# LANL-Bioinformatics/KWAGE

Hardware: AMD Instinct MI355X
Metric: G k-mer·sample bit-tests/sec (+ achieved HBM GB/s of the gather kernel in `roofline`) (higher is better)
Workload: dtype u32

## Files before the change

kwage_amd/csrc/engine.hip:

```cpp
#include <hip/hip_runtime.h>
#include <hip/hip_ext.h>

#include <algorithm>
#include <chrono>
#include <cmath>
#include <cstdio>
#include <cctype>
#include <cstring>
#include <new>
#include <string>
#include <thread>
#include <vector>

#include <unistd.h>

#include "host.hpp"
#include "engine_state.hpp"
#include "kernels.hpp"

using namespace kwage;


struct TuningName { const char *name; int64_t Tuning::*field; };
static const TuningName TUNING_NAMES[] = {
// ... 78 lines not shown
	chunk_q.reserve(n);
	chunk_t0.reserve(n);
	for(uint32_t i = 0; i < n; ++i){
		const uint64_t npos = L->h_pos_off[i + 1] - L->h_pos_off[i];
		const bool is_long = npos && (1ull << host_table_log2(npos)) > KM_LDS_SLOTS;
		if(!is_long || npos <= KM_CHUNK){ chunk_q.push_back(i); chunk_t0.push_back(0); continue; }
		L->multi_chunk = true;
		for(uint64_t t0 = 0; t0 < npos; t0 += KM_CHUNK){ chunk_q.push_back(i); chunk_t0.push_back(t0); }
	}
	if(chunk_q.size() > 0x7FFFFFFFull){ return fail(KWAGE_ERR_ARG, "batch too large for one k-mer launch"); }
	L->n_chunks = chunk_q.size();
	L->pool = &b->ctx->batch_pool;
	HIP_TRY(L->pool->take(std::max<size_t>(chunk_q.size(), 1)*sizeof(uint32_t), (void**)&L->d_chunk_q, &L->cap_chunk_q));
	HIP_TRY(L->pool->take(std::max<size_t>(chunk_q.size(), 1)*sizeof(uint64_t), (void**)&L->d_chunk_t0, &L->cap_chunk_t0));
	HIP_TRY(L->pool->take(((size_t)n + 1)*sizeof(uint64_t), (void**)&L->d_pos_off, &L->cap_pos_off));
	HIP_TRY(L->pool->take(std::max<size_t>(n, 1)*sizeof(uint64_t), (void**)&L->d_tab_off, &L->cap_tab_off));
	hipStream_t us = b->ctx->upload_stream;
	if(L->n_chunks){
		HIP_TRY(hipMemcpyAsync(L->d_chunk_q, chunk_q.data(), chunk_q.size()*sizeof(uint32_t), hipMemcpyHostToDevice, us));
		HIP_TRY(hipMemcpyAsync(L->d_chunk_t0, chunk_t0.data(), chunk_t0.size()*sizeof(uint64_t), hipMemcpyHostToDevice, us));
	}
	HIP_TRY(hipMemcpyAsync(L->d_pos_off, L->h_pos_off.data(), ((size_t)n + 1)*sizeof(uint64_t), hipMemcpyHostToDevice, us));
	if(n){ HIP_TRY(hipMemcpyAsync(L->d_tab_off, tab_off.data(), (size_t)n*sizeof(uint64_t), hipMemcpyHostToDevice, us)); }
	HIP_TRY(hipStreamSynchronize(us));
	L->total_pos = L->h_pos_off[n];
	L->max_pos = maxp;
	L->table_slots = slots;
	*out = L.get();
	b->layouts.push_back(std::move(L));
	return KWAGE_OK;
}

int launch_kmer_stage(Slot *sl, const kwage_params &p, kwage_batch *b, const KmerLayout *L, float threshold,
                      uint32_t *d_rows, uint64_t *d_kmers)
{
	int rc = layout_result(sl, b->n, 0, false);
	if(rc){ return rc; }
	if(L->table_slots){
		if((rc = sl->tables.reserve(L->table_slots*sizeof(uint64_t)))){ return rc; }
		HIP_TRY(hipMemsetAsync(sl->tables.p, 0xFF, L->table_slots*sizeof(uint64_t), sl->stream));
	}
	HIP_TRY(hipMemsetAsync(sl->d_counters, 0, 4*sizeof(uint64_t), sl->stream));
	if(b->n == 0){ return KWAGE_OK; }

	KmerArgs a;
	a.seqs = b->d_seqs;
	a.seq_off = b->d_seq_off;
	a.pos_off = L->d_pos_off;
	a.tab_off = L->d_tab_off;
	a.g_tables = (unsigned long long*)sl->tables.p;
	a.k = p.kmer_len;
	a.num_hash = p.num_hash;
	a.row_mask = (p.log_2_filter_len >= 32) ? 0xFFFFFFFFu : ((1u << p.log_2_filter_len) - 1u);
	a.threshold = threshold;
	a.complete_match = (threshold == 1.0f) ? 1 : 0;
	a.rows = d_rows;
	a.kmers_out = d_kmers;
	a.nkmer = sl->d_nkmer;
	a.qthr = sl->d_qthr;
	a.total_kmers = nullptr;
	a.shared_lg = 0;
	a.bloom_bits = nullptr;
	a.chunk_q = L->d_chunk_q;
	a.chunk_t0 = L->d_chunk_t0;
	if(L->multi_chunk){
		HIP_TRY(hipMemsetAsync(sl->d_nkmer, 0, (size_t)b->n*sizeof(uint32_t), sl->stream));
	}
	uint32_t slots = 64;
	while(slots < KM_LDS_SLOTS && slots < 2*L->max_pos){ slots *= 2; }
	a.lds_slots = slots;
	const uint32_t threads = (L->max_pos <= 192) ? 64 : (L->max_pos <= 768) ? 128 : KM_THREADS;
	hipLaunchKernelGGL(kmer_kernel, dim3((uint32_t)L->n_chunks), dim3(threads), (size_t)slots*sizeof(uint64_t), sl->stream, a);
	HIP_TRY(hipGetLastError());
	if(L->multi_chunk){
		hipLaunchKernelGGL(kmer_finish_kernel, dim3((b->n + 255)/256), dim3(256), 0, sl->stream, a, b->n);
		HIP_TRY(hipGetLastError());
	}
	return KWAGE_OK;
}

struct StageEvents { hipEvent_t start = nullptr, stop = nullptr; };

#define KW_GATHER_LAUNCH(ge, first, last, kernel, grid, block, lds, stream, ...) \
	hipExtLaunchKernelGGL(kernel, grid, block, (uint32_t)(lds), stream, (first) ? (ge).start : nullptr, (last) ? (ge).stop : nullptr, 0u, __VA_ARGS__)

static const uint32_t WALK_MIN_ROWS_PER_WAVE = 64;
static const uint32_t WALK_WAVES_PER_CU = 8;

uint32_t search_blocks(const SearchArgs &a)
{
	const uint64_t tiles = (uint64_t)a.n_queries*a.segs*a.chunks;
	return (uint32_t)((tiles + 3)/4);
}

struct WalkShape { uint32_t wgs, wg_waves; size_t lds; };
static const size_t WALK_PAD_LDS = 100*1024;

WalkShape walk_shape(const Tuning &tn, uint64_t want_waves, uint64_t ncu)
{
	WalkShape w;
	const bool pinned = tn.walk_one_wg_per_cu && want_waves == ncu*WALK_WG_WAVES;
	w.wg_waves = pinned ? (uint32_t)WALK_WG_WAVES : 4u;
	w.wgs = (uint32_t)((want_waves + w.wg_waves - 1)/w.wg_waves);
	w.lds = pinned ? WALK_PAD_LDS : 0;
	return w;
}
// ... 184 lines not shown
	ra.seg_rows = (uint32_t)std::max<uint64_t>(ra.seg_rows, (max_rows + 65535)/65536);
	ra.min_rows = (uint32_t)std::max<int64_t>(tn.refine_min_rows, 1);
	ra.max_groups = (uint32_t)std::min<int64_t>(std::max<int64_t>(tn.refine_max_groups, 0), 16);
	uint64_t items = std::min<uint64_t>(std::max<uint64_t>(8ull*a.n_queries, 1u << 16), 1u << 20);
	items = std::max<uint64_t>(std::min<uint64_t>(items, (256ull << 20)/item_bytes), 1024);
	uint64_t units = std::min<uint64_t>(std::max<uint64_t>(32*total_rows/ra.seg_rows, 1u << 18), 1u << 25);
	if(unit_bytes){ units = std::max<uint64_t>(std::min<uint64_t>(units, (512ull << 20)/unit_bytes), 4096); }
	if(tn.refine_list_cap > 0){ items = units = (uint64_t)std::min<int64_t>(tn.refine_list_cap, 1 << 20); }
	uint64_t clusters = items;
	if(exact_units){ clusters = exact_clusters; items = exact_items; units = exact_units; }
	if(exact_units && tn.refine_list_cap > 0){ clusters = items = units = (uint64_t)std::min<int64_t>(tn.refine_list_cap, 1 << 20); }
	const uint64_t tiles_per_wave = (tiles + screen_waves - 1)/std::max<uint64_t>(screen_waves, 1);
	auto list = [&](uint64_t cap, uint64_t stat_max, uint64_t chunk_max) {
		RefineList ls;
		ls.cap = (uint32_t)cap;
		ls.stat = (tn.refine_static && !exact_units) ? (uint32_t)std::min<uint64_t>(stat_max, cap/2/std::max<uint64_t>(screen_waves, 1)) : 0u;
		ls.base = (uint32_t)(ls.stat*screen_waves);
		ls.chunk = exact_units ? 1u : (uint32_t)std::max<uint64_t>(1, std::min<uint64_t>(chunk_max, tiles_per_wave/4));
		return ls;
	};
	ra.lc = list(clusters, 32, 32);
	ra.li = list(items, 64, 64);
	ra.lu = list(units, 256, 256);
	if((rc = sl->ref_counters.reserve(8*sizeof(uint32_t)))){ return rc; }
	if((rc = sl->ref_clusters.reserve(clusters*sizeof(RefineCluster)))){ return rc; }
	if((rc = sl->ref_masks.reserve(items*item_bytes))){ return rc; }
	if((rc = sl->ref_units.reserve(units*sizeof(RefineUnit)))){ return rc; }
	if(unit_bytes && (rc = sl->ref_slab.reserve(units*unit_bytes))){ return rc; }
	ra.counters = (uint32_t*)sl->ref_counters.p;
	ra.clusters = (RefineCluster*)sl->ref_clusters.p;
	ra.masks = (uint32_t*)sl->ref_masks.p;
	ra.units = (RefineUnit*)sl->ref_units.p;
	ra.slab = (uint32_t*)sl->ref_slab.p;
	HIP_TRY(hipMemsetAsync(ra.counters, 0, 8*sizeof(uint32_t), gs));
	sl->ref_base[0] = ra.lc.base; sl->ref_base[1] = ra.li.base; sl->ref_base[2] = ra.lu.base;
	sl->ref_cap[0] = ra.lc.cap; sl->ref_cap[1] = ra.li.cap; sl->ref_cap[2] = ra.lu.cap;
	ra.queue_batch = (uint32_t)std::max<uint64_t>(1, std::min<uint64_t>(16, tiles/(8*std::max<uint64_t>(screen_waves, 1))));
	ra.check_every = (tn.count_screen_check == 16 || tn.count_screen_check == 32 || tn.count_screen_check == 64) ? (uint32_t)tn.count_screen_check : 8u;
	out->refine_wgs = (uint32_t)(ncu*8);
	out->emit_wgs = (uint32_t)(ncu*4);
	return KWAGE_OK;
}

uint32_t count_screen_blocks_per_cu(uint32_t planes, uint32_t nh)
{
	static int cache[3][5] = {};
	const int pi = (planes <= 7) ? 0 : (planes <= 10) ? 1 : 2, ni = (int)std::min(std::max(nh, 1u), 5u) - 1;
	if(cache[pi][ni] == 0){
		int nb = 0;
		hipError_t e = hipErrorUnknown;
#define KWAGE_OCC_NH(P, N) case N: e = hipOccupancyMaxActiveBlocksPerMultiprocessor(&nb, count_screen_kernel<P, N>, SEARCH_THREADS, 0); break;
#define KWAGE_OCC_P(I, P) case I: switch(ni + 1){ KWAGE_OCC_NH(P, 1) KWAGE_OCC_NH(P, 2) KWAGE_OCC_NH(P, 3) KWAGE_OCC_NH(P, 4) default: KWAGE_OCC_NH(P, 5) } break;
		switch(pi){ KWAGE_OCC_P(0, 7) KWAGE_OCC_P(1, 10) default: KWAGE_OCC_P(2, 14) }
#undef KWAGE_OCC_P
#undef KWAGE_OCC_NH
		if(e != hipSuccess || nb <= 0){ (void)hipGetLastError(); nb = 2; }
		cache[pi][ni] = nb;
	}
	return (uint32_t)cache[pi][ni];
}

int launch_search_stage(Slot *sl, kwage_group *g, kwage_batch *b, const KmerLayout *L, float threshold, uint32_t flags,
                        kwage_hit *d_hits, uint64_t cap, unsigned long long *hit_count, hipStream_t gs, const StageEvents &ge)
{
	const Tuning &tn = g->ctx->tune;
	const uint64_t ncu = (uint64_t)std::max(g->ctx->ncu, 1);
	SearchArgs a;
// ... 329 lines not shown
				case 20: rc = launch_count_combine<20>(a, seg_planes, gs, ge); break;
				default: rc = launch_count_combine<32>(a, seg_planes, gs, ge); break;
			}
			if(rc){ return rc; }
		}
	}
	HIP_TRY(hipGetLastError());
	return KWAGE_OK;
}

static const uint64_t SPEC_HITS = 8192;
static const uint64_t SORT_SCRATCH_KEEP = 1ull << 30;

struct SearchOutcome {
	uint64_t staged_hits = 0;
	uint64_t n_hits = 0;
	uint64_t total_kmers = 0;
	float kmer_ms = 0, search_ms = 0;
	uint32_t launches = 0;
	char kernel_name[64] = "";
};

int enqueue_search_and_copy(Slot *sl)
{
	int rc;
	kwage_group *g = sl->g;
	kwage_batch *b = sl->b;
	const bool timing = (sl->flags & KWAGE_SEARCH_TIMING) != 0;
	const bool own = (sl->ext_hits == nullptr && sl->ext_cap == 0);
	const uint64_t cap = own ? sl->hit_cap : sl->ext_cap;
	kwage_hit *d_hits = own ? sl->d_hits : sl->ext_hits;
	if(b->n && g->num_columns){
		hipStream_t gs = g->ctx->gather_stream;
		if(sl->n_runs){ HIP_TRY(hipMemsetAsync(sl->runs.p, 0, sl->n_runs*sizeof(unsigned long long), sl->stream)); }
		HIP_TRY(hipEventRecord(sl->kmer_done, sl->stream));
		HIP_TRY(hipStreamWaitEvent(gs, sl->kmer_done, 0));
		if(sl->append && sl->append_reset){ HIP_TRY(hipMemsetAsync(sl->ext_count, 0, sizeof(uint64_t), gs)); }
		const bool ride = g->ctx->tune.ext_launch_events != 0;
		StageEvents ge;
		if(ride){ ge.start = timing ? sl->ev[2] : nullptr; ge.stop = sl->gather_done; }
		else if(timing){ HIP_TRY(hipEventRecord(sl->ev[2], gs)); }
		unsigned long long *hit_count = sl->append ? (unsigned long long*)sl->ext_count : (unsigned long long*)sl->d_counters;
		if((rc = launch_search_stage(sl, g, b, sl->lay, sl->threshold, sl->flags, d_hits, cap, hit_count, gs, ge))){ return rc; }
		if(!ride){ HIP_TRY(hipEventRecord(sl->gather_done, gs)); }
		HIP_TRY(hipStreamWaitEvent(sl->stream, sl->gather_done, 0));
		++sl->launches;
	}
	else if(sl->append && sl->append_reset){
		hipStream_t gs = g->ctx->gather_stream;
		HIP_TRY(hipMemsetAsync(sl->ext_count, 0, sizeof(uint64_t), gs));
		HIP_TRY(hipEventRecord(sl->gather_done, gs));
		HIP_TRY(hipStreamWaitEvent(sl->stream, sl->gather_done, 0));
	}
	if(sl->append){
		HIP_TRY(hipMemcpyAsync(sl->d_counters, sl->ext_count, sizeof(uint64_t), hipMemcpyDeviceToDevice, sl->stream));
	}
	else if(sl->ext_count){
		HIP_TRY(hipMemcpyAsync(sl->ext_count, sl->d_counters, sizeof(uint64_t), hipMemcpyDeviceToDevice, sl->stream));
	}
	sl->staged_hits = own ? std::min<uint64_t>(SPEC_HITS, cap) : 0;
	const uint64_t bytes = sl->head_bytes + sl->staged_hits*sizeof(kwage_hit);
	if((rc = sl->h_stage.reserve(bytes))){ return rc; }
	HIP_TRY(hipMemcpyAsync(sl->h_stage.p, sl->result.p, bytes, hipMemcpyDeviceToHost, sl->stream));
	return KWAGE_OK;
}

int submit_search(Slot *sl, kwage_group *g, kwage_batch *b, float threshold, uint32_t flags,
// ... 1 lines not shown
                  bool append = false, bool append_reset = false, uint32_t col_base = 0)
{
	kwage_ctx *ctx = g->ctx;
	int rc;
	if(sl->busy){ return fail(KWAGE_ERR_STATE, "search slot is busy: collect the pending search first"); }
	if(!g->finalized){ return fail(KWAGE_ERR_STATE, "kwage_group_finalize() must be called before searching"); }
	if(b->ctx != ctx){ return fail(KWAGE_ERR_ARG, "batch and group belong to different contexts"); }
	if(!(threshold > 0.0f) || threshold > 1.0f){
		return fail(KWAGE_ERR_ARG, "search threshold must satisfy 0 < t <= 1");
	}
	if((rc = set_device(ctx))){ return rc; }
	const KmerLayout *L = nullptr;
	if((rc = batch_prepare(b, g->params.kmer_len, &L))){ return rc; }
	if(L->max_pos*g->params.num_hash > 0xFFFFFFFFull){
		return fail(KWAGE_ERR_ARG, "a query of %llu k-mer positions x %u hash functions exceeds 2^32 rows", (unsigned long long)L->max_pos, g->params.num_hash);
	}
	if((rc = sl->rows.reserve(std::max<uint64_t>(L->total_pos*g->params.num_hash, 1)*sizeof(uint32_t)))){ return rc; }
	sl->g = g; sl->b = b; sl->lay = L; sl->threshold = threshold; sl->flags = flags;
	sl->ext_hits = ext_hits; sl->ext_cap = ext_cap; sl->ext_count = ext_count;
	sl->append = append; sl->append_reset = append_reset; sl->col_base = col_base;
	sl->launches = 0;
	sl->n_runs = 0;
	sl->runs_per_query = 0;
	if(ext_hits == nullptr && ext_cap == 0 && b->n && g->num_columns){
		const uint64_t kib = (g->stride/16 + WAVE - 1)/WAVE;
		const uint64_t walk_tile = (uint64_t)std::min<int64_t>(std::max<int64_t>(ctx->tune.walk_tile_kib, 1), 16);
		sl->runs_per_query = (uint32_t)(kib + (kib + walk_tile - 1)/walk_tile + 4);
		sl->n_runs = (uint64_t)b->n*sl->runs_per_query;
		if((rc = sl->runs.reserve(sl->n_runs*sizeof(unsigned long long)))){ return rc; }
	}

	const bool timing_kmer = (flags & KWAGE_SEARCH_TIMING) && (flags & KWAGE_SEARCH_TIMING_KMER);
	if(timing_kmer){ HIP_TRY(hipEventRecord(sl->ev[0], sl->stream)); }
	if((rc = launch_kmer_stage(sl, g->params, b, L, threshold, (uint32_t*)sl->rows.p, nullptr))){ return rc; }
	if(g->d_row_map && b->n){
		const uint64_t per_q = std::max<uint64_t>(1, (L->max_pos*g->params.num_hash + 4095)/4096);
		const uint64_t wgs_per_q = std::min<uint64_t>(per_q, std::max<uint64_t>(1, 0x7FFFFFFFull/b->n));
		hipLaunchKernelGGL(remap_rows_kernel, dim3((uint32_t)(b->n*wgs_per_q)), dim3(256), 0, sl->stream, (uint32_t*)sl->rows.p, L->d_pos_off, sl->d_nkmer,
		                   g->params.num_hash, g->d_row_map, (uint32_t)g->h_row_map.size(), (unsigned long long*)sl->d_counters + 2, (uint32_t)wgs_per_q);
		HIP_TRY(hipGetLastError());
	}
	if(timing_kmer){ HIP_TRY(hipEventRecord(sl->ev[1], sl->stream)); }
	if((rc = enqueue_search_and_copy(sl))){ return rc; }
	sl->busy = true;
	return KWAGE_OK;
}

int collect_search_steps(Slot *sl, SearchOutcome *out);

int collect_search(Slot *sl, SearchOutcome *out)
{
	if(!sl->busy){ return fail(KWAGE_ERR_STATE, "no pending search in this slot"); }
	kwage_ctx *ctx = sl->g->ctx;
	const int rc = collect_search_steps(sl, out);
	if(rc){
		(void)hipStreamSynchronize(ctx->gather_stream);
		(void)hipStreamSynchronize(sl->stream);
		(void)hipGetLastError();
	}
	return rc;
}

int collect_search_steps(Slot *sl, SearchOutcome *out)
{
	if(!sl->busy){ return fail(KWAGE_ERR_STATE, "no pending search in this slot"); }
	kwage_ctx *ctx = sl->g->ctx;
	int rc = set_device(ctx);
// ... 654 lines not shown
}

namespace {

int run_shared_kmer_pass(kwage_ctx *ctx, const kwage_params &p, kwage_batch *b, uint32_t *d_bloom_bits, uint64_t *distinct)
{
	Slot *sl = &ctx->slot[0];
	if(sl->busy){ return fail(KWAGE_ERR_STATE, "a search is pending on this context"); }
	const KmerLayout *L = nullptr;
	int rc = batch_prepare(b, p.kmer_len, &L);
	if(rc){ return rc; }
	if((rc = layout_result(sl, b->n, 0, false))){ return rc; }
	uint32_t lg = 10;
	while((1ull << lg) < 2*std::max<uint64_t>(L->total_pos, 1)){ ++lg; }
	if(ctx->tune.shared_table_log2 > 0){ lg = std::max<uint32_t>(lg, (uint32_t)ctx->tune.shared_table_log2); }
	if(lg > 36){ return fail(KWAGE_ERR_ARG, "too many k-mer positions for one sample"); }
	if((rc = sl->tables.reserve((1ull << lg)*sizeof(uint64_t)))){ return rc; }
	HIP_TRY(hipMemsetAsync(sl->tables.p, 0xFF, (1ull << lg)*sizeof(uint64_t), ctx->stream));
	HIP_TRY(hipMemsetAsync(sl->d_counters, 0, 4*sizeof(uint64_t), ctx->stream));
	if(b->n){
		KmerArgs a;
		a.seqs = b->d_seqs; a.seq_off = b->d_seq_off; a.pos_off = L->d_pos_off; a.tab_off = L->d_tab_off;
		a.g_tables = (unsigned long long*)sl->tables.p;
		a.k = p.kmer_len; a.num_hash = p.num_hash;
		a.row_mask = (p.log_2_filter_len >= 32) ? 0xFFFFFFFFu : ((1u << p.log_2_filter_len) - 1u);
		a.threshold = 1.0f; a.complete_match = 1;
		a.rows = nullptr; a.kmers_out = nullptr;
		a.nkmer = sl->d_nkmer; a.qthr = sl->d_qthr;
		a.total_kmers = (unsigned long long*)sl->d_counters + 1;
		a.shared_lg = lg;
		a.bloom_bits = d_bloom_bits;
		a.chunk_q = nullptr; a.chunk_t0 = nullptr;
		a.lds_slots = 0;
		hipLaunchKernelGGL(kmer_kernel, dim3(b->n), dim3(KM_THREADS), 0, ctx->stream, a);
		HIP_TRY(hipGetLastError());
	}
	uint64_t h[2] = {0, 0};
	HIP_TRY(hipMemcpyAsync(h, sl->d_counters, sizeof(h), hipMemcpyDeviceToHost, ctx->stream));
	HIP_TRY(hipStreamSynchronize(ctx->stream));
	if(distinct){ *distinct = h[1]; }
	return KWAGE_OK;
}

}

extern "C" int kwage_count_distinct_kmers(kwage_ctx *ctx, kwage_batch *b, uint32_t kmer_len, uint64_t *count)
{
	if(!ctx || !b || !count){ return fail(KWAGE_ERR_ARG, "kwage_count_distinct_kmers: NULL argument"); }
	if(b->ctx != ctx){ return fail(KWAGE_ERR_ARG, "kwage_count_distinct_kmers: batch belongs to another context"); }
	kwage_params p = {kmer_len, 1, 0, KWAGE_HASH_MURMUR32};
	int rc = check_params(&p);
	if(rc){ return rc; }
	if((rc = set_device(ctx))){ return rc; }
	return run_shared_kmer_pass(ctx, p, b, nullptr, count);
}

extern "C" int kwage_bloom_bits_from_batch(kwage_ctx *ctx, const kwage_params *params, kwage_batch *b,
                                           void *bits_out, uint64_t *distinct)
{
	if(!ctx || !params || !b || !bits_out){ return fail(KWAGE_ERR_ARG, "kwage_bloom_bits_from_batch: NULL argument"); }
	if(b->ctx != ctx){ return fail(KWAGE_ERR_ARG, "kwage_bloom_bits_from_batch: batch belongs to another context"); }
	int rc = check_params(params);
	if(rc){ return rc; }
	if((rc = set_device(ctx))){ return rc; }
	const uint64_t nbytes = ((1ull << params->log_2_filter_len) + 7)/8;
	const uint64_t alloc = (nbytes + 3)/4*4;
	DevBuf bits;
// ... 44 lines not shown
```

kwage_amd/csrc/engine_state.hpp:

```cpp
#ifndef KWAGE_AMD_ENGINE_STATE_HPP
#define KWAGE_AMD_ENGINE_STATE_HPP

#include <hip/hip_runtime.h>

#include <algorithm>
#include <deque>
#include <memory>
#include <mutex>
#include <vector>

#include "internal.h"

#define HIP_TRY(expr)                                                                          \
	do {                                                                                       \
		hipError_t _e = (expr);                                                                \
		if(_e != hipSuccess){                                                                  \
			return fail(KWAGE_ERR_DEVICE, "%s failed: %s (%s:%d)", #expr, hipGetErrorString(_e), \
			            __FILE__, __LINE__);                                                   \
		}                                                                                      \
	} while(0)

struct kwage_group;
struct kwage_batch;
struct kwage_ctx;
// ... 168 lines not shown
		cached.clear();
	}
};


struct Slot {
	hipStream_t stream = nullptr;
	hipEvent_t ev[4] = {nullptr, nullptr, nullptr, nullptr};
	hipEvent_t kmer_done = nullptr;
	hipEvent_t gather_done = nullptr;
	DevBuf rows, tables, partial;
	DevBuf result;
	uint64_t *d_counters = nullptr;
	uint32_t *d_nkmer = nullptr, *d_qthr = nullptr;
	kwage_hit *d_hits = nullptr;
	uint64_t hit_cap = 0, head_bytes = 0;
	PinBuf h_stage;
	DevBuf sort_scratch;
	DevBuf runs;
	uint64_t n_runs = 0;
	uint32_t runs_per_query = 0;
	bool busy = false;
	kwage_group *g = nullptr;
	kwage_batch *b = nullptr;
	const KmerLayout *lay = nullptr;
	float threshold = 1.0f;
	uint32_t flags = 0;
	uint32_t launches = 0;
	char kernel_name[64] = "";
	DevBuf walk_or, walk_done;
	DevBuf band_rows, band_loc, band_or, band_state;
	DevBuf cwalk_slab, cwalk_arrived;
	DevBuf ref_counters, ref_clusters, ref_masks, ref_units, ref_slab;
	DevBuf trunc_dev;
	PinBuf trunc_host;
	uint32_t ref_base[3] = {0, 0, 0}, ref_cap[3] = {0, 0, 0};
	uint64_t staged_hits = 0;
	kwage_hit *ext_hits = nullptr;
	uint64_t ext_cap = 0;
	uint64_t *ext_count = nullptr;
	bool append = false, append_reset = false;
	uint32_t col_base = 0;
};

struct Tuning {
	int64_t walk = 4;
	int64_t walk_min_rows = -1;
	int64_t walk_max_kib = 16;
	int64_t walk_tile_kib = 16;
	int64_t walk_min_kib = 2;
	int64_t walk_waves = 0;
	int64_t walk_one_wg_per_cu = 1;
	int64_t walk_bands = -1;
	int64_t walk_bands_min_gib = 48;
	int64_t and_vec = 0;
	int64_t and_wide_min_kib = 16;
	int64_t and_wide = 1;
	int64_t narrow = 1;
	int64_t force_segs = 0;
	int64_t ee_refine = 1;
	int64_t refine_seg_rows = 32;
	int64_t refine_min_rows = 32;
	int64_t refine_max_groups = 4;
	int64_t refine_unroll = 8;
	int64_t screen_wpc = 20;
	int64_t count_screen_wpc = 32;
// ... 120 lines not shown
```

kwage_amd/csrc/kernels.hpp:

```cpp
#ifndef KWAGE_AMD_KERNELS_HPP
#define KWAGE_AMD_KERNELS_HPP

#include <hip/hip_runtime.h>
#include <stdint.h>

#include "kwage_amd.h"
#include "kmer_device.hpp"

namespace kwage {

static constexpr int WAVE = 64;
static constexpr int KM_THREADS = 256;
static constexpr uint32_t KM_LDS_SLOTS = 4096;
static constexpr uint32_t KM_CHUNK = 1024;
static constexpr uint64_t KM_EMPTY = ~0ull;
static constexpr int SEARCH_THREADS = 256;


__device__ __forceinline__ uint32_t table_log2(uint64_t npos)
{
	uint32_t lg = 6;
	while((1ull << lg) < 2*npos){ ++lg; }
	return lg;
}

template <typename PTR>
__device__ __forceinline__ bool set_insert(PTR tab, uint32_t lg, uint64_t w)
{
	const uint64_t mask = (1ull << lg) - 1ull;
	uint64_t s = ((w * 0x9E3779B97F4A7C15ull) >> (64 - lg)) & mask;
	while(true){
		const unsigned long long old = atomicCAS(&tab[s], (unsigned long long)KM_EMPTY, (unsigned long long)w);
		if(old == KM_EMPTY){ return true; }
		if(old == w){ return false; }
		s = (s + 1) & mask;
	}
}

struct KmerArgs {
	const char *seqs;
	const uint64_t *seq_off;
	const uint64_t *pos_off;
	const uint64_t *tab_off;
	unsigned long long *g_tables;
	uint32_t k, num_hash, row_mask;
	float threshold;
	int complete_match;
	uint32_t *rows;
	uint64_t *kmers_out;
	uint32_t *nkmer;
	uint32_t *qthr;
	unsigned long long *total_kmers;
	uint32_t lds_slots;
	uint32_t shared_lg;
	uint32_t *bloom_bits;
	const uint32_t *chunk_q;
	const uint64_t *chunk_t0;
};

template <bool LDS_TAB, bool MULTI, typename TAB>
__device__ __forceinline__ void kmer_body(const KmerArgs &a, uint32_t q, uint64_t s0, uint64_t len,
                                          uint64_t t_begin, uint64_t t_end, TAB tab, uint32_t lg,
                                          uint8_t *codes, uint32_t *count, uint32_t *tile_base)
{
	const uint32_t k = a.k;
	const uint64_t base = a.pos_off[q];
	const uint64_t kmask = (k == 32) ? ~0ull : ((1ull << (2*k)) - 1ull);

	if(LDS_TAB){
		for(uint32_t i = threadIdx.x; i < (1u << lg); i += blockDim.x){ tab[i] = KM_EMPTY; }
	}
	if(threadIdx.x == 0){ *count = 0; }
	__syncthreads();

	for(uint64_t t0 = t_begin; t0 < t_end; t0 += blockDim.x){
		const uint32_t nchar = (uint32_t)min((uint64_t)(blockDim.x + k - 1), len - t0);
		for(uint32_t i = threadIdx.x; i < nchar; i += blockDim.x){
			codes[i] = (uint8_t)base_code(a.seqs[s0 + t0 + i]);
		}
		__syncthreads();

		const uint64_t p = t0 + threadIdx.x;
		bool fresh = false;
		uint64_t canon = 0;
		if(p < t_end){
			uint64_t w = 0;
			uint32_t bad = 0;
			for(uint32_t j = 0; j < k; ++j){
				const uint32_t c = codes[threadIdx.x + j];
				bad |= c >> 2;
				w = (w << 2) | (c & 3u);
			}
			if(!bad){
				w &= kmask;
// ... 14 lines not shown
			__syncthreads();
			idx += *tile_base;
		}
		else if(fresh){ idx = atomicAdd(count, 1u); }
		if(fresh){
			if(a.kmers_out){ a.kmers_out[base + idx] = canon; }
			if(a.bloom_bits){
				MurmurKeys mk;
				murmur_keys(canon, k, mk);
				for(uint32_t h = 0; h < a.num_hash; ++h){
					const uint32_t bit = murmur_finish(mk, k, h) & a.row_mask;
					atomicOr(a.bloom_bits + (bit >> 5), 1u << (bit & 31));
				}
			}
			if(a.rows){
				MurmurKeys mk;
				murmur_keys(canon, k, mk);
				for(uint32_t h = 0; h < a.num_hash; ++h){
					a.rows[(base + idx)*a.num_hash + h] = murmur_finish(mk, k, h) & a.row_mask;
				}
			}
		}
		__syncthreads();
	}

	if(!MULTI && threadIdx.x == 0){
		const uint32_t n = *count;
		a.nkmer[q] = n;
		a.qthr[q] = a.complete_match ? 0u : (uint32_t)__fmul_rn(a.threshold, (float)n);
		if(n && a.total_kmers){ atomicAdd(a.total_kmers, (unsigned long long)n); }
	}
}

__global__ __launch_bounds__(KM_THREADS) void kmer_kernel(KmerArgs a)
{
	extern __shared__ __attribute__((aligned(16))) unsigned long long lds_tab[];
	__shared__ uint8_t codes[KM_THREADS + KWAGE_MAX_WORD_LEN];
	__shared__ uint32_t count, tile_base;

	const uint32_t q = a.chunk_q ? a.chunk_q[blockIdx.x] : blockIdx.x;
	const uint64_t t_begin = a.chunk_q ? a.chunk_t0[blockIdx.x] : 0;
	const uint64_t s0 = a.seq_off[q];
	const uint64_t len = a.seq_off[q + 1] - s0;
	const uint64_t npos = (len >= a.k) ? (len - a.k + 1) : 0;

	if(npos == 0){
		if(threadIdx.x == 0){ a.nkmer[q] = 0; a.qthr[q] = 0; }
		return;
	}

	if(a.shared_lg){
		kmer_body<false, false>(a, q, s0, len, 0, npos, a.g_tables, a.shared_lg, codes, &count, &tile_base);
		return;
	}
	const uint32_t lg = table_log2(npos);
	if((1ull << lg) <= a.lds_slots){
		kmer_body<true, false>(a, q, s0, len, 0, npos, lds_tab, lg, codes, &count, &tile_base);
	}
	else if(npos <= KM_CHUNK){
		kmer_body<false, false>(a, q, s0, len, 0, npos, a.g_tables + a.tab_off[q], lg, codes, &count, &tile_base);
	}
	else{
		kmer_body<false, true>(a, q, s0, len, t_begin, min(npos, t_begin + (uint64_t)KM_CHUNK), a.g_tables + a.tab_off[q], lg, codes, &count, &tile_base);
	}
}

__global__ __launch_bounds__(256) void kmer_finish_kernel(KmerArgs a, uint32_t n_queries)
{
	const uint32_t q = blockIdx.x*blockDim.x + threadIdx.x;
	if(q < n_queries){ a.qthr[q] = a.complete_match ? 0u : (uint32_t)__fmul_rn(a.threshold, (float)a.nkmer[q]); }
}

__global__ __launch_bounds__(256) void remap_rows_kernel(uint32_t *rows, const uint64_t *pos_off, const uint32_t *nkmer, uint32_t num_hash,
                                                         const uint32_t *map, uint32_t map_len, unsigned long long *missing, uint32_t wgs_per_query)
{
	const uint32_t q = blockIdx.x / wgs_per_query, part = blockIdx.x % wgs_per_query;
	uint32_t *rq = rows + pos_off[q]*num_hash;
	const uint64_t n = (uint64_t)nkmer[q]*num_hash;
	for(uint64_t e = (uint64_t)part*blockDim.x + threadIdx.x; e < n; e += (uint64_t)wgs_per_query*blockDim.x){
		const uint32_t r = rq[e];
		uint32_t lo = 0, hi = map_len;
		while(lo < hi){
			const uint32_t mid = lo + (hi - lo)/2;
			if(map[mid] < r){ lo = mid + 1; } else { hi = mid; }
		}
		if(lo < map_len && map[lo] == r){ rq[e] = lo; }
		else{ rq[e] = 0; atomicAdd(missing, 1ull); }
	}
}

struct SearchArgs {
	const uint8_t *db;
	uint64_t stride;
	uint32_t units_per_row;
	const uint8_t *valid;
	const uint32_t *rows;
// ... 1660 lines not shown
```

kwage_amd/csrc/topk.hip:

```cpp
#include <hip/hip_runtime.h>
#include <stdint.h>

#include <algorithm>
#include <cstddef>
#include <cstdio>
#include <cstring>
#include <memory>
#include <new>
#include <vector>

#include "kwage_amd.h"
#include "engine_state.hpp"
#include "pool_blocks.hpp"

namespace topk_dev {
#include "kernels.hpp"
#include "topk_kernels.hpp"
}

namespace dev = topk_dev::kwage;

namespace kwage {
namespace {

// ... 172 lines not shown
	d_missing = (unsigned long long*)(((uintptr_t)(d_out_n + std::max<uint32_t>(n, 1)) + 7) & ~(uintptr_t)7);
	if((rc = blocks.take(std::max<uint64_t>((uint64_t)n*k, 1)*sizeof(kwage_hit), &d_out))){ return rc; }
	HIP_TRY(hipMemsetAsync(d_missing, 0, sizeof(unsigned long long), s));

	if(timing_kmer){ HIP_TRY(hipEventRecord(ev.ev[0], s)); }
	if(n){
		if(L->table_slots){
			if((rc = blocks.take(L->table_slots*sizeof(uint64_t), &d_tables))){ return rc; }
			HIP_TRY(hipMemsetAsync(d_tables, 0xFF, L->table_slots*sizeof(uint64_t), s));
		}
		dev::KmerArgs ka;
		ka.seqs = b->d_seqs;
		ka.seq_off = b->d_seq_off;
		ka.pos_off = L->d_pos_off;
		ka.tab_off = L->d_tab_off;
		ka.g_tables = d_tables;
		ka.k = g->params.kmer_len;
		ka.num_hash = nh;
		ka.row_mask = (g->params.log_2_filter_len >= 32) ? 0xFFFFFFFFu : ((1u << g->params.log_2_filter_len) - 1u);
		ka.threshold = threshold;
		ka.complete_match = 0;
		ka.rows = d_rows;
		ka.kmers_out = nullptr;
		ka.nkmer = d_nkmer;
		ka.qthr = d_qthr;
		ka.total_kmers = nullptr;
		ka.lds_slots = 64;
		while(ka.lds_slots < dev::KM_LDS_SLOTS && ka.lds_slots < 2*L->max_pos){ ka.lds_slots *= 2; }
		ka.shared_lg = 0;
		ka.bloom_bits = nullptr;
		ka.chunk_q = L->d_chunk_q;
		ka.chunk_t0 = L->d_chunk_t0;
		if(L->multi_chunk){ HIP_TRY(hipMemsetAsync(d_nkmer, 0, (size_t)n*sizeof(uint32_t), s)); }
		const uint32_t threads = (L->max_pos <= 192) ? 64 : (L->max_pos <= 768) ? 128 : dev::KM_THREADS;
		hipLaunchKernelGGL(dev::kmer_kernel, dim3((uint32_t)L->n_chunks), dim3(threads), (size_t)ka.lds_slots*sizeof(uint64_t), s, ka);
		HIP_TRY(hipGetLastError());
		if(L->multi_chunk){
			hipLaunchKernelGGL(dev::kmer_finish_kernel, dim3((n + 255)/256), dim3(256), 0, s, ka, n);
			HIP_TRY(hipGetLastError());
		}
		if(g->d_row_map){
			const uint64_t per_q = std::max<uint64_t>(1, (L->max_pos*nh + 4095)/4096);
			const uint64_t wgs_per_q = std::min<uint64_t>(per_q, std::max<uint64_t>(1, 0x7FFFFFFFull/n));
			hipLaunchKernelGGL(dev::remap_rows_kernel, dim3((uint32_t)(n*wgs_per_q)), dim3(256), 0, s, d_rows, L->d_pos_off, d_nkmer,
			                   nh, g->d_row_map, (uint32_t)g->h_row_map.size(), d_missing, (uint32_t)wgs_per_q);
			HIP_TRY(hipGetLastError());
		}
	}
	if(timing_kmer){ HIP_TRY(hipEventRecord(ev.ev[1], s)); }

	char kernel_name[64] = "";
	uint32_t launches = 0;
	if(timing){ HIP_TRY(hipEventRecord(ev.ev[2], s)); }
	if(n && g->num_columns){
		dev::SearchArgs a;
		memset(&a, 0, sizeof(a));
		a.db = g->d_bits;
		a.stride = g->stride;
		a.units_per_row = (uint32_t)(g->stride/16);
		a.valid = g->d_valid;
		a.rows = d_rows;
		a.num_hash = nh;
		a.chunks = (a.units_per_row + dev::WAVE - 1)/dev::WAVE;
		const uint32_t planes = topk_planes_for(L->max_pos);
		const uint64_t cand_per_q = (uint64_t)a.chunks*k*sizeof(unsigned long long);
		uint32_t slice = (uint32_t)std::max<uint64_t>(1, std::min<uint64_t>(n, CAND_BYTES_PER_SLICE/cand_per_q));
		a.n_queries = slice;
		topk_segments(a, L->max_pos, ctx->tune.force_segs);
// ... 211 lines not shown
```

Before: 51730.

## Pack sequence bits with wave ballots in k-mer kernel and fold scratch memsets into it

Rewrites the k-mer extraction kernel to first pack the query bases into 2-bit words plus an invalid-base bitmap in LDS using wave ballots. Each thread then extracts its k-mer window with shifts instead of walking a per-tile code buffer, and the old serial path is kept only for the bloom kernel. The kernel also zeroes the slot counters, refine counters and run buffers itself, so the separate hipMemsetAsync calls before the gather are skipped. This trades a few launch overheads and serial code scanning for extra LDS use and per-round block syncs in the multi-chunk path.

```diff
diff --git a/kwage_amd/csrc/engine.hip b/kwage_amd/csrc/engine.hip
--- a/kwage_amd/csrc/engine.hip
+++ b/kwage_amd/csrc/engine.hip
@@ -134,16 +134,19 @@
 }
 
 int launch_kmer_stage(Slot *sl, const kwage_params &p, kwage_batch *b, const KmerLayout *L, float threshold,
-                      uint32_t *d_rows, uint64_t *d_kmers)
-{
+                      uint32_t *d_rows, uint64_t *d_kmers, bool search_scratch = false)
+{
+	sl->ref_cleared = sl->runs_cleared = false;
 	int rc = layout_result(sl, b->n, 0, false);
 	if(rc){ return rc; }
 	if(L->table_slots){
 		if((rc = sl->tables.reserve(L->table_slots*sizeof(uint64_t)))){ return rc; }
 		HIP_TRY(hipMemsetAsync(sl->tables.p, 0xFF, L->table_slots*sizeof(uint64_t), sl->stream));
 	}
-	HIP_TRY(hipMemsetAsync(sl->d_counters, 0, 4*sizeof(uint64_t), sl->stream));
-	if(b->n == 0){ return KWAGE_OK; }
+	if(b->n == 0){
+		HIP_TRY(hipMemsetAsync(sl->d_counters, 0, 4*sizeof(uint64_t), sl->stream));
+		return KWAGE_OK;
+	}
 
 	KmerArgs a;
 	a.seqs = b->d_seqs;
@@ -165,15 +168,27 @@
 	a.bloom_bits = nullptr;
 	a.chunk_q = L->d_chunk_q;
 	a.chunk_t0 = L->d_chunk_t0;
+	a.clear[0] = (unsigned long long*)sl->d_counters;
+	a.clear_words[0] = 4;
+	if(search_scratch){
+		if((rc = sl->ref_counters.reserve(8*sizeof(uint32_t)))){ return rc; }
+		a.clear[1] = (unsigned long long*)sl->ref_counters.p;
+		a.clear_words[1] = 4;
+		if(sl->n_runs){
+			a.clear[2] = (unsigned long long*)sl->runs.p;
+			a.clear_words[2] = sl->n_runs;
+		}
+	}
 	if(L->multi_chunk){
 		HIP_TRY(hipMemsetAsync(sl->d_nkmer, 0, (size_t)b->n*sizeof(uint32_t), sl->stream));
 	}
 	uint32_t slots = 64;
 	while(slots < KM_LDS_SLOTS && slots < 2*L->max_pos){ slots *= 2; }
 	a.lds_slots = slots;
-	const uint32_t threads = (L->max_pos <= 192) ? 64 : (L->max_pos <= 768) ? 128 : KM_THREADS;
-	hipLaunchKernelGGL(kmer_kernel, dim3((uint32_t)L->n_chunks), dim3(threads), (size_t)slots*sizeof(uint64_t), sl->stream, a);
+	hipLaunchKernelGGL(kmer_kernel, dim3((uint32_t)L->n_chunks), dim3(kmer_threads(L->max_pos)), (size_t)slots*sizeof(uint64_t), sl->stream, a);
 	HIP_TRY(hipGetLastError());
+	sl->ref_cleared = search_scratch;
+	sl->runs_cleared = search_scratch && sl->n_runs;
 	if(L->multi_chunk){
 		hipLaunchKernelGGL(kmer_finish_kernel, dim3((b->n + 255)/256), dim3(256), 0, sl->stream, a, b->n);
 		HIP_TRY(hipGetLastError());
@@ -424,7 +439,8 @@
 	ra.masks = (uint32_t*)sl->ref_masks.p;
 	ra.units = (RefineUnit*)sl->ref_units.p;
 	ra.slab = (uint32_t*)sl->ref_slab.p;
-	HIP_TRY(hipMemsetAsync(ra.counters, 0, 8*sizeof(uint32_t), gs));
+	if(!sl->ref_cleared){ HIP_TRY(hipMemsetAsync(ra.counters, 0, 8*sizeof(uint32_t), gs)); }
+	sl->ref_cleared = false;
 	sl->ref_base[0] = ra.lc.base; sl->ref_base[1] = ra.li.base; sl->ref_base[2] = ra.lu.base;
 	sl->ref_cap[0] = ra.lc.cap; sl->ref_cap[1] = ra.li.cap; sl->ref_cap[2] = ra.lu.cap;
 	ra.queue_batch = (uint32_t)std::max<uint64_t>(1, std::min<uint64_t>(16, tiles/(8*std::max<uint64_t>(screen_waves, 1))));
@@ -820,7 +836,8 @@
 	kwage_hit *d_hits = own ? sl->d_hits : sl->ext_hits;
 	if(b->n && g->num_columns){
 		hipStream_t gs = g->ctx->gather_stream;
-		if(sl->n_runs){ HIP_TRY(hipMemsetAsync(sl->runs.p, 0, sl->n_runs*sizeof(unsigned long long), sl->stream)); }
+		if(sl->n_runs && !sl->runs_cleared){ HIP_TRY(hipMemsetAsync(sl->runs.p, 0, sl->n_runs*sizeof(unsigned long long), sl->stream)); }
+		sl->runs_cleared = false;
 		HIP_TRY(hipEventRecord(sl->kmer_done, sl->stream));
 		HIP_TRY(hipStreamWaitEvent(gs, sl->kmer_done, 0));
 		if(sl->append && sl->append_reset){ HIP_TRY(hipMemsetAsync(sl->ext_count, 0, sizeof(uint64_t), gs)); }
@@ -888,7 +905,7 @@
 
 	const bool timing_kmer = (flags & KWAGE_SEARCH_TIMING) && (flags & KWAGE_SEARCH_TIMING_KMER);
 	if(timing_kmer){ HIP_TRY(hipEventRecord(sl->ev[0], sl->stream)); }
-	if((rc = launch_kmer_stage(sl, g->params, b, L, threshold, (uint32_t*)sl->rows.p, nullptr))){ return rc; }
+	if((rc = launch_kmer_stage(sl, g->params, b, L, threshold, (uint32_t*)sl->rows.p, nullptr, true))){ return rc; }
 	if(g->d_row_map && b->n){
 		const uint64_t per_q = std::max<uint64_t>(1, (L->max_pos*g->params.num_hash + 4095)/4096);
 		const uint64_t wgs_per_q = std::min<uint64_t>(per_q, std::max<uint64_t>(1, 0x7FFFFFFFull/b->n));
@@ -1609,7 +1626,7 @@
 		a.bloom_bits = d_bloom_bits;
 		a.chunk_q = nullptr; a.chunk_t0 = nullptr;
 		a.lds_slots = 0;
-		hipLaunchKernelGGL(kmer_kernel, dim3(b->n), dim3(KM_THREADS), 0, ctx->stream, a);
+		hipLaunchKernelGGL(kmer_bloom_kernel, dim3(b->n), dim3(KM_THREADS), 0, ctx->stream, a);
 		HIP_TRY(hipGetLastError());
 	}
 	uint64_t h[2] = {0, 0};
diff --git a/kwage_amd/csrc/engine_state.hpp b/kwage_amd/csrc/engine_state.hpp
--- a/kwage_amd/csrc/engine_state.hpp
+++ b/kwage_amd/csrc/engine_state.hpp
@@ -224,6 +224,7 @@
 	DevBuf band_rows, band_loc, band_or, band_state;
 	DevBuf cwalk_slab, cwalk_arrived;
 	DevBuf ref_counters, ref_clusters, ref_masks, ref_units, ref_slab;
+	bool ref_cleared = false, runs_cleared = false;
 	DevBuf trunc_dev;
 	PinBuf trunc_host;
 	uint32_t ref_base[3] = {0, 0, 0}, ref_cap[3] = {0, 0, 0};
diff --git a/kwage_amd/csrc/kernels.hpp b/kwage_amd/csrc/kernels.hpp
--- a/kwage_amd/csrc/kernels.hpp
+++ b/kwage_amd/csrc/kernels.hpp
@@ -11,8 +11,10 @@
 
 static constexpr int WAVE = 64;
 static constexpr int KM_THREADS = 256;
+static constexpr int KM_MAX_THREADS = 256;
 static constexpr uint32_t KM_LDS_SLOTS = 4096;
 static constexpr uint32_t KM_CHUNK = 1024;
+static constexpr uint32_t KM_PACK_WORDS = 2*((KM_LDS_SLOTS/2 + KWAGE_MAX_WORD_LEN + 32 + 63)/64);
 static constexpr uint64_t KM_EMPTY = ~0ull;
 static constexpr int SEARCH_THREADS = 256;
 
@@ -22,6 +24,11 @@
 	uint32_t lg = 6;
 	while((1ull << lg) < 2*npos){ ++lg; }
 	return lg;
+}
+
+__host__ __device__ inline uint32_t kmer_threads(uint64_t max_pos)
+{
+	return (max_pos <= 192) ? 64u : (max_pos <= 768) ? 128u : (uint32_t)KM_MAX_THREADS;
 }
 
 template <typename PTR>
@@ -56,10 +63,12 @@
 	uint32_t *bloom_bits;
 	const uint32_t *chunk_q;
 	const uint64_t *chunk_t0;
+	unsigned long long *clear[3] = {nullptr, nullptr, nullptr};
+	uint64_t clear_words[3] = {0, 0, 0};
 };
 
 template <bool LDS_TAB, bool MULTI, typename TAB>
-__device__ __forceinline__ void kmer_body(const KmerArgs &a, uint32_t q, uint64_t s0, uint64_t len,
+__device__ __forceinline__ void kmer_body_serial(const KmerArgs &a, uint32_t q, uint64_t s0, uint64_t len,
                                           uint64_t t_begin, uint64_t t_end, TAB tab, uint32_t lg,
                                           uint8_t *codes, uint32_t *count, uint32_t *tile_base)
 {
@@ -140,11 +149,133 @@
 	}
 }
 
-__global__ __launch_bounds__(KM_THREADS) void kmer_kernel(KmerArgs a)
-{
-	extern __shared__ __attribute__((aligned(16))) unsigned long long lds_tab[];
+__global__ __launch_bounds__(KM_THREADS) void kmer_bloom_kernel(KmerArgs a)
+{
 	__shared__ uint8_t codes[KM_THREADS + KWAGE_MAX_WORD_LEN];
 	__shared__ uint32_t count, tile_base;
+	const uint32_t q = blockIdx.x;
+	const uint64_t s0 = a.seq_off[q];
+	const uint64_t len = a.seq_off[q + 1] - s0;
+	const uint64_t npos = (len >= a.k) ? (len - a.k + 1) : 0;
+	if(npos == 0){
+		if(threadIdx.x == 0){ a.nkmer[q] = 0; a.qthr[q] = 0; }
+		return;
+	}
+	kmer_body_serial<false, false>(a, q, s0, len, 0, npos, a.g_tables, a.shared_lg, codes, &count, &tile_base);
+}
+
+__device__ __forceinline__ uint64_t spread_bits(uint32_t v)
+{
+	uint64_t x = v;
+	x = (x | (x << 16)) & 0x0000FFFF0000FFFFull;
+	x = (x | (x << 8)) & 0x00FF00FF00FF00FFull;
+	x = (x | (x << 4)) & 0x0F0F0F0F0F0F0F0Full;
+	x = (x | (x << 2)) & 0x3333333333333333ull;
+	x = (x | (x << 1)) & 0x5555555555555555ull;
+	return x;
+}
+
+__device__ __forceinline__ void kmer_stage_packed(const char *seq, uint64_t nb, uint64_t *pw, uint32_t *pb)
+{
+	const uint32_t lane = threadIdx.x & (WAVE - 1), nwaves = blockDim.x/WAVE;
+	const uint32_t steps = (uint32_t)min((nb + 32 + 63)/64, (uint64_t)KM_PACK_WORDS/2);
+	for(uint32_t st = threadIdx.x/WAVE; st < steps; st += nwaves){
+		const uint64_t i = (uint64_t)st*64 + lane;
+		const uint32_t c = (i < nb) ? base_code(seq[i]) : 4u;
+		const uint64_t lo = __ballot(c & 1u), hi = __ballot((c >> 1) & 1u), bad = __ballot(c >> 2);
+		if(lane < 2){
+			const uint32_t sh = 32*lane;
+			pw[2*st + lane] = (spread_bits(__brev((uint32_t)(hi >> sh))) << 1) | spread_bits(__brev((uint32_t)(lo >> sh)));
+			pb[2*st + lane] = __brev((uint32_t)(bad >> sh));
+		}
+	}
+}
+
+template <bool LDS_TAB, bool MULTI, typename TAB>
+__device__ __forceinline__ void kmer_body(const KmerArgs &a, uint32_t q, uint64_t s0, uint64_t len, uint64_t t_begin, uint64_t t_end,
+                                          TAB tab, uint32_t lg, uint64_t *pw, uint32_t *pb, uint32_t *count, uint32_t *round_base)
+{
+	const uint32_t k = a.k;
+	const uint32_t lane = threadIdx.x & (WAVE - 1);
+	const uint64_t base = a.pos_off[q];
+	const uint64_t span = t_end - t_begin;
+	if(LDS_TAB){
+		ulonglong2 *t2 = reinterpret_cast<ulonglong2*>(tab);
+		const ulonglong2 e = make_ulonglong2(KM_EMPTY, KM_EMPTY);
+		for(uint32_t i = threadIdx.x; i < (1u << lg)/2; i += blockDim.x){ t2[i] = e; }
+	}
+	if(threadIdx.x == 0){ *count = 0; }
+	kmer_stage_packed(a.seqs + s0 + t_begin, min(span + k - 1, len - t_begin), pw, pb);
+	__syncthreads();
+
+	for(uint64_t r0 = 0; r0 < span; r0 += blockDim.x){
+		const uint32_t p = (uint32_t)r0 + threadIdx.x;
+		bool fresh = false;
+		uint64_t canon = 0;
+		if(r0 + threadIdx.x < span){
+			const uint32_t j = p >> 5, o = p & 31u;
+			const uint64_t bb = ((uint64_t)pb[j] << 32) | pb[j + 1];
+			if(((bb << o) >> (64 - k)) == 0){
+				const uint64_t w0 = pw[j], w1 = pw[j + 1];
+				const uint64_t win = o ? ((w0 << (2*o)) | (w1 >> (64 - 2*o))) : w0;
+				const uint64_t w = win >> (64 - 2*k);
+				const uint64_t rc = revcomp2(w, k);
+				canon = (w < rc) ? w : rc;
+				fresh = set_insert(tab, lg, canon);
+			}
+		}
+		const uint64_t mask = __ballot(fresh);
+		const uint32_t rank = (uint32_t)__popcll(mask & ((1ull << lane) - 1ull));
+		uint32_t wave_base = 0;
+		if(mask){
+			const uint32_t leader = (uint32_t)__ffsll((unsigned long long)mask) - 1u;
+			if(lane == leader){ wave_base = atomicAdd(count, (uint32_t)__popcll(mask)); }
+			wave_base = __shfl(wave_base, (int)leader);
+		}
+		uint32_t idx = wave_base + rank;
+		if(MULTI){
+			__syncthreads();
+			if(threadIdx.x == 0){
+				const uint32_t n_new = *count;
+				*round_base = n_new ? atomicAdd(a.nkmer + q, n_new) : 0u;
+				*count = 0;
+			}
+			__syncthreads();
+			idx += *round_base;
+		}
+		if(fresh){
+			if(a.kmers_out){ a.kmers_out[base + idx] = canon; }
+			if(a.rows){
+				MurmurKeys mk;
+				murmur_keys(canon, k, mk);
+				for(uint32_t h = 0; h < a.num_hash; ++h){
+					a.rows[(base + idx)*a.num_hash + h] = murmur_finish(mk, k, h) & a.row_mask;
+				}
+			}
+		}
+	}
+
+	if(!MULTI){
+		__syncthreads();
+		if(threadIdx.x == 0){
+			const uint32_t n = *count;
+			a.nkmer[q] = n;
+			a.qthr[q] = a.complete_match ? 0u : (uint32_t)__fmul_rn(a.threshold, (float)n);
+			if(n && a.total_kmers){ atomicAdd(a.total_kmers, (unsigned long long)n); }
+		}
+	}
+}
+
+__global__ __launch_bounds__(KM_MAX_THREADS) void kmer_kernel(KmerArgs a)
+{
+	extern __shared__ __attribute__((aligned(16))) unsigned long long lds_tab[];
+	__shared__ uint64_t pw[KM_PACK_WORDS];
+	__shared__ uint32_t pb[KM_PACK_WORDS];
+	__shared__ uint32_t count, round_base;
+
+	for(int c = 0; c < 3; ++c){
+		for(uint64_t i = (uint64_t)blockIdx.x*blockDim.x + threadIdx.x; i < a.clear_words[c]; i += (uint64_t)gridDim.x*blockDim.x){ a.clear[c][i] = 0ull; }
+	}
 
 	const uint32_t q = a.chunk_q ? a.chunk_q[blockIdx.x] : blockIdx.x;
 	const uint64_t t_begin = a.chunk_q ? a.chunk_t0[blockIdx.x] : 0;
@@ -157,19 +288,15 @@
 		return;
 	}
 
-	if(a.shared_lg){
-		kmer_body<false, false>(a, q, s0, len, 0, npos, a.g_tables, a.shared_lg, codes, &count, &tile_base);
-		return;
-	}
 	const uint32_t lg = table_log2(npos);
 	if((1ull << lg) <= a.lds_slots){
-		kmer_body<true, false>(a, q, s0, len, 0, npos, lds_tab, lg, codes, &count, &tile_base);
+		kmer_body<true, false>(a, q, s0, len, 0, npos, lds_tab, lg, pw, pb, &count, &round_base);
 	}
 	else if(npos <= KM_CHUNK){
-		kmer_body<false, false>(a, q, s0, len, 0, npos, a.g_tables + a.tab_off[q], lg, codes, &count, &tile_base);
+		kmer_body<false, false>(a, q, s0, len, 0, npos, a.g_tables + a.tab_off[q], lg, pw, pb, &count, &round_base);
 	}
 	else{
-		kmer_body<false, true>(a, q, s0, len, t_begin, min(npos, t_begin + (uint64_t)KM_CHUNK), a.g_tables + a.tab_off[q], lg, codes, &count, &tile_base);
+		kmer_body<false, true>(a, q, s0, len, t_begin, min(npos, t_begin + (uint64_t)KM_CHUNK), a.g_tables + a.tab_off[q], lg, pw, pb, &count, &round_base);
 	}
 }
 
diff --git a/kwage_amd/csrc/topk.hip b/kwage_amd/csrc/topk.hip
--- a/kwage_amd/csrc/topk.hip
+++ b/kwage_amd/csrc/topk.hip
@@ -228,8 +228,7 @@
 		ka.chunk_q = L->d_chunk_q;
 		ka.chunk_t0 = L->d_chunk_t0;
 		if(L->multi_chunk){ HIP_TRY(hipMemsetAsync(d_nkmer, 0, (size_t)n*sizeof(uint32_t), s)); }
-		const uint32_t threads = (L->max_pos <= 192) ? 64 : (L->max_pos <= 768) ? 128 : dev::KM_THREADS;
-		hipLaunchKernelGGL(dev::kmer_kernel, dim3((uint32_t)L->n_chunks), dim3(threads), (size_t)ka.lds_slots*sizeof(uint64_t), s, ka);
+		hipLaunchKernelGGL(dev::kmer_kernel, dim3((uint32_t)L->n_chunks), dim3(dev::kmer_threads(L->max_pos)), (size_t)ka.lds_slots*sizeof(uint64_t), s, ka);
 		HIP_TRY(hipGetLastError());
 		if(L->multi_chunk){
 			hipLaunchKernelGGL(dev::kmer_finish_kernel, dim3((n + 255)/256), dim3(256), 0, s, ka, n);
```

Result: no change. 51930 (median of 6 runs) (+0.4%).
